# ccalantzis/BRDF

Hardware: AMD Instinct MI355X
Metric: BRDF residual-evals/sec (1 M samples, Ward 3-param), whole job; rel-err vs CPU levmar in `parity` (higher is better)
Workload: dtype f64

## Files before the change

brdf_amd/csrc/resident_fit_impl.h:

```cpp
#pragma once
#include <type_traits>

#if defined(BRDF_STAMPS)
#include <hip/hip_runtime.h>
static __device__ long long g_rlm_stamps[8];
static __device__ long long g_rlm_last;
#endif
#if defined(BRDF_STAMPS) && defined(__HIP_DEVICE_COMPILE__)
#define LM_STAMP(i) do { if (blockIdx.x == 0) { const long long now_ = clock64(); if ((i) != 0) g_rlm_stamps[i] += now_ - g_rlm_last; g_rlm_last = now_; } } while (0)
#endif
#include "batch_fit.h"
#include "stream_fit.h"

namespace brdf {

constexpr int kRThreads = 512;
constexpr int kRSpt = 8;
constexpr int kRTile = kRThreads * kRSpt;
constexpr int kRCap = kRTile;
constexpr int kRowWords = 2 * kSlots;
constexpr int kRowStride = 256;
constexpr int kRedCols = kRThreads / 4;
constexpr long long kSpinBudgetTicks = 200000000LL;

typedef unsigned long long u64;

struct ResidentCtl {
  unsigned abort;
  unsigned domain_bad;
  unsigned pad[30];
};

struct ResidentCtx {
  const double *c0, *c1, *c2, *x;
  u64 *rows;
  u64 *groups;
  ResidentCtl *ctl;
  unsigned launch_id;
  double p0[kM], opts[5], lb[kM], ub[kM], dscl[kM];
  int itmax, has_opts, has_lb, has_ub, has_dscl, want_covar, multi, analytic;
  int chain;
  int spec_jac;
  int dif_fused;
  Mailbox *mbox;
  int n;
  unsigned tag_base;
  long long spin_ticks;
  int sabotage_epoch;
  int replicas;
  long long *trace;
  int trace_epoch;
};

template <int METHOD>
using RMachine = typename std::conditional<METHOD == 0, DifMachine<kM>, typename std::conditional<METHOD == 1, BcMachine<kM>, DerMachine<kM>>::type>::type;

__device__ __forceinline__ double read_lane(double v, int lane) {
  const int lo = __builtin_amdgcn_readlane(__double2loint(v), lane);
  const int hi = __builtin_amdgcn_readlane(__double2hiint(v), lane);
  return __hiloint2double(hi, lo);
}

__device__ __forceinline__ void acc_normal_eq_fma(const double *j, double e, double *jtj6, double *jte3) {
  jtj6[0] = fma(j[0], j[0], jtj6[0]);
  jtj6[1] = fma(j[0], j[1], jtj6[1]);
  jtj6[2] = fma(j[1], j[1], jtj6[2]);
  jtj6[3] = fma(j[0], j[2], jtj6[3]);
  jtj6[4] = fma(j[1], j[2], jtj6[4]);
  jtj6[5] = fma(j[2], j[2], jtj6[5]);
  jte3[0] = fma(j[0], e, jte3[0]);
  jte3[1] = fma(j[1], e, jte3[1]);
  jte3[2] = fma(j[2], e, jte3[2]);
}
__device__ __forceinline__ double div_by(double x, double d, double r) {
  const double q = x * r;
  return fma(fma(-q, d, x), r, q);
}

#ifdef BRDF_STAMPS
#define RSTAMP(i) do { const long long now_ = clock64(); st_[i] += now_ - last_; last_ = now_; } while (0)
#define RTRACE(ctx_, epoch_, slot_, val_) do { if ((ctx_).trace && (int)(epoch_) == (ctx_).trace_epoch && (threadIdx.x & 63) == 0) (ctx_).trace[blockIdx.x * 8 + (slot_)] = (long long)(val_); } while (0)
#else
#define RSTAMP(i) do {} while (0)
#define RTRACE(ctx_, epoch_, slot_, val_) do {} while (0)
#endif

constexpr int kFc0 = 0, kFx = 1, kFq1 = 2, kFq2 = 3, kFhx = 4, kFwrk = 5, kFtb = 6;
template <int METHOD>
constexpr int sample_fields() { return METHOD == 0 ? 7 : 4; }

template <int METHOD>
struct RegSamples {
  static constexpr bool kUnrolled = true;
  double v[sample_fields<METHOD>()][kRSpt];
  __device__ __forceinline__ double get(int f, int k) const { return v[f][k]; }
  __device__ __forceinline__ void set(int f, int k, double x) { v[f][k] = x; }
};
template <int METHOD>
struct LdsSamples {
  static constexpr bool kUnrolled = false;
  double *base;
  __device__ __forceinline__ double get(int f, int k) const { return base[(f * kRSpt + k) * kWave]; }
  __device__ __forceinline__ void set(int f, int k, double x) { base[(f * kRSpt + k) * kWave] = x; }
};

template <bool UNROLLED, class F>
__device__ __forceinline__ void for_samples(int nk, F &&f) {
  if constexpr (UNROLLED) {
#pragma unroll
    for (int k = 0; k < kRSpt; ++k)
      if (k < nk) f(k);
  } else {
#pragma unroll 2
    for (int k = 0; k < nk; ++k) f(k);
  }
}

constexpr int kGroup = 16;
constexpr int kMaxGroups = 16;
constexpr int kReplicas = 8;
constexpr size_t kBlockGranules = (size_t)kRowWords * kGroup;
constexpr size_t kRowsGranules = 2 * (size_t)kMaxGroups * kBlockGranules;
constexpr size_t kGroupsGranules = 2 * (size_t)kReplicas * kBlockGranules;

typedef unsigned int u32x4 __attribute__((ext_vector_type(4)));
constexpr int kCacheSc1 = 16;
__device__ __forceinline__ __amdgpu_buffer_rsrc_t table_rsrc(const u64 *p, size_t granules) {
  return __builtin_amdgcn_make_buffer_rsrc(const_cast<u64 *>(p), 0, (int)(granules * sizeof(u64)), 0x00027000);
}
__device__ __forceinline__ void put_cell(__amdgpu_buffer_rsrc_t t, unsigned cell, unsigned tag, double v) {
  const u32x4 d = {(unsigned)__double2loint(v), tag, (unsigned)__double2hiint(v), tag};
  __builtin_amdgcn_raw_buffer_store_b128(d, t, (int)(cell * 16u), 0, kCacheSc1);
}

struct RowPublish {
  const u64 *rows;
  unsigned cell0;
  unsigned tag;
  bool on;
  bool withhold;
};

template <int NS, bool MAX = true, bool PUB = false>
__device__ __forceinline__ void worker_reduce(const double *acc, double mx, double *buf, double *out, const RowPublish &pub, long long *st_,
                                              long long &last_) {
  const int lane = threadIdx.x & (kWave - 1);
  const int wave = threadIdx.x >> 6;
  double v[NS + 1];
#pragma unroll
  for (int k = 0; k < NS; ++k) {
    double t = acc[k];
    t = t + dpp_move<0x111, 0xf, 0xf>(t, 0.0);
    t = t + dpp_move<0x112, 0xf, 0xf>(t, 0.0);
    v[k] = t;
  }
  if constexpr (MAX) {
    double t = mx;
    t = fmax(t, dpp_move<0x111, 0xf, 0xf>(t, 0.0));
    t = fmax(t, dpp_move<0x112, 0xf, 0xf>(t, 0.0));
    v[NS] = t;
  }
  constexpr int NV = NS + (MAX ? 1 : 0);
  if ((threadIdx.x & 3) == 3) {
#pragma unroll
    for (int k = 0; k < NV; ++k) buf[k * kRedCols + (threadIdx.x >> 2)] = v[k];
  }
  __syncthreads();
  RSTAMP(6);
  {
    constexpr int NW = kRThreads / kWave;
    const int k0 = wave, k1 = wave + NW;
    const bool has0 = k0 < NV, has1 = k1 < NV;
    double s0 = 0.0, s1 = 0.0;
    if (has0) {
      const double *src = buf + k0 * kRedCols;
      s0 = (k0 < NS || !MAX) ? src[lane] + src[lane + kWave] : fmax(src[lane], src[lane + kWave]);
    }
    if (has1) {
      const double *src = buf + k1 * kRedCols;
      s1 = (k1 < NS || !MAX) ? src[lane] + src[lane + kWave] : fmax(src[lane], src[lane + kWave]);
    }
    const bool max0 = MAX && has0 && k0 == NS, max1 = MAX && has1 && k1 == NS;
    if (!max0 && !max1) {
      wave_reduce2_to_last<OpSum, OpSum>(s0, s1);
    } else if (max1) {
      wave_reduce2_to_last<OpSum, OpMax>(s0, s1);
    } else {
      wave_reduce2_to_last<OpMax, OpSum>(s0, s1);
    }
    if constexpr (PUB) {
      if (pub.on) {
        if (lane == kWave - 1 && !pub.withhold) {
          const __amdgpu_buffer_rsrc_t rows = table_rsrc(pub.rows, kRowsGranules);
          if (has0) put_cell(rows, pub.cell0 + (max0 ? kSums : k0) * kGroup, pub.tag, s0);
          if (has1) put_cell(rows, pub.cell0 + (max1 ? kSums : k1) * kGroup, pub.tag, s1);
        }
        return;
      }
    }
    if (lane == kWave - 1) {
      if (has0) out[max0 ? kSums : k0] = s0;
      if (has1) out[max1 ? kSums : k1] = s1;
    }
  }
  __syncthreads();
}

__device__ __forceinline__ RowPublish row_publish(const ResidentCtx &ctx, unsigned epoch) {
  const unsigned grp = blockIdx.x / kGroup;
  return RowPublish{ctx.rows, ((epoch & 1u) * kMaxGroups + grp) * (kSlots * kGroup) + blockIdx.x % kGroup, ctx.tag_base + epoch + 1u, gridDim.x > 1,
                    (int)epoch == ctx.sabotage_epoch && blockIdx.x == gridDim.x - 1};
}

template <int NS, bool MAX = true>
__device__ __forceinline__ constexpr bool slot_used(int v) { return v < NS || (MAX && v == kSums); }

template <int NS, bool MAX = true, class Ctx>
__device__ __forceinline__ bool gather_block(const Ctx &ctx, __amdgpu_buffer_rsrc_t t, unsigned first, unsigned tag, int ncols,
                                             double (&val)[4], unsigned *polls) {
  const int lane = threadIdx.x & (kWave - 1);
  const int col = lane & 15, r = lane >> 4;
  const long long t0 = (long long)wall_clock64();
  for (unsigned spins = 0;; ++spins) {
    u32x4 d[4];
    bool ready = true;
#pragma unroll
    for (int j = 0; j < 4; ++j) {
      d[j] = u32x4{0u, tag, 0u, tag};
      if ((4 * j < NS) || (MAX && 4 * j <= kSums && kSums < 4 * j + 4)) {
        const int v = 4 * j + r;
        if (slot_used<NS, MAX>(v) && col < ncols) d[j] = __builtin_amdgcn_raw_buffer_load_b128(t, (int)((first + v * kGroup + col) * 16u), 0, kCacheSc1);
      }
    }
#pragma unroll
    for (int j = 0; j < 4; ++j) ready = ready && d[j].y == tag && d[j].w == tag;
    if (__all(ready)) {
#pragma unroll
      for (int j = 0; j < 4; ++j) val[j] = __hiloint2double((int)d[j].z, (int)d[j].x);
      *polls = spins;
      return true;
    }
    if ((spins & 63u) == 63u) {
      if (__hip_atomic_load(&ctx.ctl->abort, __ATOMIC_RELAXED, __HIP_MEMORY_SCOPE_AGENT) == ctx.launch_id ||
          (long long)wall_clock64() - t0 > ctx.spin_ticks) {
        __hip_atomic_store(&ctx.ctl->abort, ctx.launch_id, __ATOMIC_RELAXED, __HIP_MEMORY_SCOPE_AGENT);
        return false;
      }
    }
    __builtin_amdgcn_s_sleep(1);
  }
}

template <int NS, bool MAX>
__device__ __forceinline__ void fold_block(double (&val)[4]) {
  const int r = (int)(threadIdx.x & (kWave - 1)) >> 4;
  double mx = 0.0;
  if constexpr (MAX) mx = row_reduce_to_last<OpMax>(val[kSums / 4]);
#pragma unroll
  for (int j = 0; j < 4; ++j)
    if ((4 * j < NS) || (MAX && j == kSums / 4)) val[j] = row_reduce_to_last<OpSum>(val[j]);
  if (MAX && r == (kSums & 3)) val[kSums / 4] = mx;
}

template <int NS, bool MAX = true, bool PUBLISHED = false, class Ctx>
__device__ __forceinline__ bool control_exchange(const Ctx &ctx, unsigned epoch, double *sums, int *s_abort,
                                                 long long *st_, long long &last_) {
  const int lane = threadIdx.x & (kWave - 1);
  const int col = lane & 15, r = lane >> 4;
  const int G = gridDim.x;
  const int grp = blockIdx.x / kGroup, ngrp = (G + kGroup - 1) / kGroup;
  const int members = min(kGroup, G - grp * kGroup);
  const int leader = grp * kGroup + (grp & 7) % members;
  const unsigned tag = ctx.tag_base + epoch + 1u;
  constexpr unsigned kBlockCells = kSlots * kGroup;
  const __amdgpu_buffer_rsrc_t rows = table_rsrc(ctx.rows, kRowsGranules), groups = table_rsrc(ctx.groups, kGroupsGranules);
  const unsigned my_rows = ((epoch & 1u) * kMaxGroups + grp) * kBlockCells;
  const unsigned my_groups = (epoch & 1u) * kReplicas * kBlockCells;
  if constexpr (!PUBLISHED) {
    const bool withhold = (int)epoch == ctx.sabotage_epoch && blockIdx.x == gridDim.x - 1;
    if (slot_used<NS, MAX>(lane) && lane <= kSums && !withhold) put_cell(rows, my_rows + lane * kGroup + blockIdx.x % kGroup, tag, sums[lane]);
  }

  double val[4];
  unsigned polls = 0;
  if ((int)blockIdx.x == leader) {
    if (!gather_block<NS, MAX>(ctx, rows, my_rows, tag, members, val, &polls)) {
      *s_abort = 1;
      return false;
    }
#ifndef BRDF_TRACE_WORKERS
    RTRACE(ctx, epoch, 6, polls + 1);
#endif
    fold_block<NS, MAX>(val);
#pragma unroll
    for (int j = 0; j < 4; ++j) {
      const double t = dpp_move<0x15F, 0xf, 0xf>(val[j], 0.0);
      const int v = 4 * j + r;
      if (slot_used<NS, MAX>(v) && col < ctx.replicas) put_cell(groups, my_groups + col * kBlockCells + v * kGroup + grp, tag, t);
    }
  }
  RSTAMP(2);
  RTRACE(ctx, epoch, 3, wall_clock64());
  if (!gather_block<NS, MAX>(ctx, groups, my_groups + (blockIdx.x % ctx.replicas) * kBlockCells, tag, ngrp, val, &polls)) {
    *s_abort = 1;
    return false;
  }
  fold_block<NS, MAX>(val);
#pragma unroll
  for (int j = 0; j < 4; ++j) {
    const int v = 4 * j + r;
    if (slot_used<NS, MAX>(v) && col == kGroup - 1) sums[v] = val[j];
  }
  __builtin_amdgcn_fence(__ATOMIC_RELEASE, "wavefront");
  __builtin_amdgcn_wave_barrier();
  RSTAMP(3);
  RTRACE(ctx, epoch, 4, wall_clock64());
#ifndef BRDF_TRACE_WORKERS
  RTRACE(ctx, epoch, 7, polls);
#endif
  return true;
}

template <int MODEL>
__device__ __forceinline__ void build_uniforms_wave(PassUniforms<MODEL> &u, const Request<kM> &r, bool need_base, bool analytic_jac) {
  using Mdl = BrdfModel<MODEL>;
  const int lane = (int)(threadIdx.x & (kWave - 1));
  if (r.kind == RQ_EVAL_MULTI) {
    u.ncand = r.nk;
    u.analytic = analytic_jac ? 1 : 0;
    if (lane < kMaxCand && lane < r.nk) {
      const double pk[kM] = {r.pk[lane][0], r.pk[lane][1], r.pk[lane][2]};
      u.lk[lane] = Mdl::lin(pk);
      u.nk[lane] = Mdl::nl(pk);
    }
    return;
  }
  if ((r.kind == RQ_JAC && !analytic_jac) || r.kind == RQ_DIF_JAC) {
    u.ncand = 0;
    u.analytic = 0;
    u.central = r.central;
    u.scal = r.scal;
    u.dp_l2 = r.dp_l2;
#pragma unroll
    for (int j = 0; j < kM; ++j) u.dp[j] = r.dp[j];
    if (lane < 1 + 2 * kM) {
      const int j = lane == 0 ? 0 : (lane - 1) % kM;
      const bool plus = lane >= 1 && lane <= kM, minus = lane > kM;
      double pp[kM];
#pragma unroll
      for (int i = 0; i < kM; ++i) {
        pp[i] = r.p[i];
        if (i == j && plus) pp[i] = r.p[i] + r.d[i];
        if (i == j && minus) pp[i] = r.p[i] - r.d[i];
      }
      const Lin l = Mdl::lin(pp);
      const Nl nn = Mdl::nl(pp);
      if (lane == 0) {
        u.l0 = l;
        u.n0 = nn;
      } else if (plus) {
        u.lp[j] = l;
        if (j == kM - 1) u.np2 = nn;
        double dj = r.d[0];
#pragma unroll
        for (int i = 1; i < kM; ++i)
          if (i == j) dj = r.d[i];
        u.dinv[j] = (r.central ? 0.5 : 1.0) / dj;
      } else {
        u.lm[j] = l;
        if (j == kM - 1) u.nm2 = nn;
      }
    }
    return;
  }
  u.build(r, need_base, analytic_jac);
}

template <int MODEL, int METHOD, bool FAST, class Store>
__device__ __forceinline__ void sweep_pass(int kind, const PassUniforms<MODEL> &u, Store &st, double *jl, int tid, int nk, int nfull, unsigned okm,
                                           bool pend, const double *dpp, double *acc, double &mx) {
  constexpr bool U = Store::kUnrolled;
  constexpr bool W2 = BrdfModel<MODEL>::prep_planes == 2;
  auto prep = [&](int k) { return Prep{st.get(kFq1, k), W2 ? st.get(kFq2, k) : 0.0}; };
  auto dead = [&](int k) { return k >= nfull && !(okm >> k & 1u); };
  switch (kind) {
  case RQ_EVAL:
    if constexpr (METHOD != 0) {
      const EvalUniforms eu{scalar_copy(u.l0), scalar_copy(u.n0), 1.0};
      for_samples<U>(nk, [&](int k) {
        const double f = model_value<MODEL, FAST>(eu, st.get(kFc0, k), prep(k));
        double e = st.get(kFx, k) - f;
        if (dead(k)) e = 0.0;
        acc[0] = fma(e, e, acc[0]);
        mx = fmax(mx, fabs(e));
      });
    }
    break;
  case RQ_SCALED:
    if constexpr (METHOD != 0) {
      const EvalUniforms eu{scalar_copy(u.l0), scalar_copy(u.n0), scalar_copy(u.scal)};
      for_samples<U>(nk, [&](int k) {
        const double f = model_value<MODEL, FAST>(eu, st.get(kFc0, k), prep(k));
        double t = (st.get(kFx, k) - f) / eu.scal;
        if (dead(k)) t = 0.0;
        acc[0] = fma(t, t, acc[0]);
      });
    }
    break;
  case RQ_EVAL_MULTI:
    if constexpr (METHOD != 2) {
      if (u.ncand == kMaxCand) {
        if constexpr (METHOD == 0) {
          for_samples<U>(nk, [&](int k) {
            const double c0 = st.get(kFc0, k), x = st.get(kFx, k);
            const Prep q = prep(k);
            const bool d = dead(k);
#pragma unroll
            for (int j0 = 0; j0 < kMaxCand; j0 += 4) {
              double e[4];
#pragma unroll
              for (int j = 0; j < 4; ++j) e[j] = x - model_value_k<MODEL, FAST>(u, j0 + j, c0, q);
#pragma unroll
              for (int j = 0; j < 4; ++j) {
                if (d) e[j] = 0.0;
                acc[j0 + j] = fma(e[j], e[j], acc[j0 + j]);
              }
            }
          });
          break;
        }
#pragma unroll
        for (int j0 = 0; j0 < kMaxCand; j0 += 4) {
          Lin l4[4];
          Nl n4[4];
#pragma unroll
          for (int j = 0; j < 4; ++j) {
            l4[j] = scalar_copy(u.lk[j0 + j]);
            n4[j] = scalar_copy(u.nk[j0 + j]);
          }
          for_samples<U>(nk, [&](int k) {
            const double c0 = st.get(kFc0, k), x = st.get(kFx, k);
            const Prep q = prep(k);
            const bool d = dead(k);
            double e[4];
#pragma unroll
            for (int j = 0; j < 4; ++j) e[j] = x - BrdfModel<MODEL>::combine(l4[j], c0, BrdfModel<MODEL>::template shape<FAST>(n4[j], c0, q));
#pragma unroll
            for (int j = 0; j < 4; ++j) {
              if (d) e[j] = 0.0;
              acc[j0 + j] = fma(e[j], e[j], acc[j0 + j]);
            }
          });
        }
        break;
      }
      for_samples<U>(nk, [&](int k) {
        const double c0 = st.get(kFc0, k), x = st.get(kFx, k);
        const Prep q = prep(k);
#pragma unroll
        for (int j = 0; j < kMaxCand; ++j)
          if (j < u.ncand) {
            double e = x - model_value_k<MODEL, FAST>(u, j, c0, q);
            if (dead(k)) e = 0.0;
            acc[j] = fma(e, e, acc[j]);
          }
      });
    }
    break;
  case RQ_JAC:
    if constexpr (METHOD != 0) {
      auto jac = [&](auto jk) {
        constexpr int JK = decltype(jk)::value;
        JacUniforms ju;
        ju.l0 = scalar_copy(u.l0);
        ju.n0 = scalar_copy(u.n0);
        ju.analytic = JK == 2;
        ju.central = JK == 1;
        if (JK == 2) {
          ju.an[0] = scalar_copy(u.an[0]);
          ju.an[1] = scalar_copy(u.an[1]);
        } else {
#pragma unroll
          for (int j = 0; j < kM; ++j) {
            ju.lp[j] = scalar_copy(u.lp[j]);
            ju.dinv[j] = scalar_copy(u.dinv[j]);
            if (JK == 1) ju.lm[j] = scalar_copy(u.lm[j]);
          }
          ju.np2 = scalar_copy(u.np2);
          if (JK == 1) ju.nm2 = scalar_copy(u.nm2);
        }
        for_samples<U>(nk, [&](int k) {
          double f0 = 0.0, j[kM];
          if (JK == 2)
            model_an_row<MODEL, FAST>(ju, st.get(kFc0, k), prep(k), f0, j);
          else if (JK == 1)
            model_fd_row_t<MODEL, FAST, true>(ju, st.get(kFc0, k), prep(k), true, f0, 0.0, false, j);
          else
            model_fd_row_t<MODEL, FAST, false>(ju, st.get(kFc0, k), prep(k), true, f0, 0.0, false, j);
          double e = st.get(kFx, k) - f0;
          if (dead(k)) e = j[0] = j[1] = j[2] = 0.0;
          acc_normal_eq_fma(j, e, acc, acc + kNL);
          acc[kNL + kM] = fma(e, e, acc[kNL + kM]);
        });
      };
      if (u.analytic)
        jac(std::integral_constant<int, 2>{});
      else if (u.central)
        jac(std::integral_constant<int, 1>{});
      else
        jac(std::integral_constant<int, 0>{});
    }
    break;
  case RQ_DIF_INIT:
    if constexpr (METHOD == 0) {
      for_samples<U>(nk, [&](int k) {
        const double h = model_value<MODEL, FAST>(u, st.get(kFc0, k), prep(k));
        st.set(kFhx, k, h);
        double e = st.get(kFx, k) - h;
        if (dead(k)) e = 0.0;
        acc[0] = fma(e, e, acc[0]);
      });
    }
    break;
  case RQ_DIF_JAC:
    if constexpr (METHOD == 0) {
      for_samples<U>(nk, [&](int k) {
        const int s = k * kRThreads + tid;
        const double h = st.get(kFhx, k);
        double f0 = 0.0, j[kM];
        model_fd_row<MODEL, FAST>(u, st.get(kFc0, k), prep(k), false, f0, h, true, j);
        double e = st.get(kFx, k) - h;
        if (dead(k)) e = j[0] = j[1] = j[2] = 0.0;
        jl[s] = j[0];
        jl[kRCap + s] = j[1];
        jl[2 * kRCap + s] = j[2];
        acc_normal_eq_fma(j, e, acc, acc + kNL);
      });
    }
    break;
  case RQ_DIF_TRIAL:
    if constexpr (METHOD == 0) {
      struct TrialUniforms {
        Lin lq;
        Nl nq;
        double dp[kM], dp_l2;
      };
      TrialUniforms tu;
      tu.lq = scalar_copy(u.lq);
      tu.nq = scalar_copy(u.nq);
#pragma unroll
      for (int j = 0; j < kM; ++j) tu.dp[j] = scalar_copy(u.dp[j]);
      tu.dp_l2 = scalar_copy(u.dp_l2);
      const double dpp_s[kM] = {scalar_copy(dpp[0]), scalar_copy(dpp[1]), scalar_copy(dpp[2])};
      const TrialUniforms &u = tu;
      const double *dpp = dpp_s;
      const double rinv = 1.0 / u.dp_l2;
      auto value_q = [&](int k) { return model_value_q<MODEL, FAST>(u, st.get(kFc0, k), prep(k)); };
      auto body = [&](int k, const double w) {
        const int s = k * kRThreads + tid;
        const double h = st.get(kFhx, k), x = st.get(kFx, k);
        double jo[kM] = {jl[s], jl[kRCap + s], jl[2 * kRCap + s]};
        if (pend) {
          const double tp = st.get(kFtb, k);
#pragma unroll
          for (int j = 0; j < kM; ++j) jo[j] = fma(tp, dpp[j], jo[j]);
          jl[s] = jo[0];
          jl[kRCap + s] = jo[1];
          jl[2 * kRCap + s] = jo[2];
        }
        double t = jo[0] * u.dp[0], jn[kM];
        t = fma(jo[1], u.dp[1], t);
        t = fma(jo[2], u.dp[2], t);
        t = div_by(w - h - t, u.dp_l2, rinv);
#pragma unroll
        for (int j = 0; j < kM; ++j) jn[j] = fma(t, u.dp[j], jo[j]);
        double en = x - w, eo = x - h;
        if (dead(k)) en = eo = jn[0] = jn[1] = jn[2] = t = 0.0;
        st.set(kFwrk, k, w);
        st.set(kFtb, k, t);
        acc[0] = fma(en, en, acc[0]);
#pragma unroll
        for (int j = 0; j < kM; ++j) acc[1 + j] = fma(jo[j], t, acc[1 + j]);
        acc[1 + kM] = fma(t, t, acc[1 + kM]);
#pragma unroll
        for (int j = 0; j < kM; ++j) acc[2 + kM + j] = fma(jn[j], en, acc[2 + kM + j]);
        acc[2 + 2 * kM] = fma(t, eo, acc[2 + 2 * kM]);
      };
      for_samples<U>(nk, [&](int k) { body(k, value_q(k)); });
    }
    break;
  default: break;
  }
}

template <int METHOD, bool PUB = false>
__device__ __forceinline__ void reduce_pass(int kind, const double *acc, double mx, double *red, double *sums, const RowPublish &pub, long long *st_,
                                            long long &last_) {
  if constexpr (METHOD == 0) {
    switch (kind) {
    case RQ_DIF_JAC: worker_reduce<SumLayout<kM>::DIF_JAC, false, PUB>(acc, mx, red, sums, pub, st_, last_); break;
    case RQ_DIF_TRIAL: worker_reduce<kTrialSums, false, PUB>(acc, mx, red, sums, pub, st_, last_); break;
    case RQ_EVAL_MULTI: worker_reduce<kMaxCand, false, PUB>(acc, mx, red, sums, pub, st_, last_); break;
    default: worker_reduce<1, false, PUB>(acc, mx, red, sums, pub, st_, last_); break;
    }
  } else {
    switch (kind) {
    case RQ_JAC: worker_reduce<SumLayout<kM>::JAC, false, PUB>(acc, mx, red, sums, pub, st_, last_); break;
    case RQ_EVAL_MULTI: worker_reduce<kMaxCand, false, PUB>(acc, mx, red, sums, pub, st_, last_); break;
    default: worker_reduce<1, METHOD == 1, PUB>(acc, mx, red, sums, pub, st_, last_); break;
    }
  }
}

#define RESIDENT_KERNEL_HEAD                                      \
  template <int MODEL, int METHOD, bool FAST, bool BATCHED>       \
  __global__ __launch_bounds__(kRThreads) void resident_fit_kernel(ResidentCtx ctx, BatchCtx bctx)
#define RESIDENT_KERNEL_FLAGS constexpr bool RAGGED = false;
#define RESIDENT_KERNEL_COUNT(fit_, stride_) (stride_)
#include "resident_fit_kernel.inc"
#undef RESIDENT_KERNEL_HEAD
#undef RESIDENT_KERNEL_FLAGS
#undef RESIDENT_KERNEL_COUNT

#define RESIDENT_KERNEL_HEAD                          \
  template <int MODEL, int METHOD, bool FAST>         \
  __global__ __launch_bounds__(kRThreads) void resident_fit_ragged_kernel(ResidentCtx ctx, RaggedBatchCtx bctx)
#define RESIDENT_KERNEL_FLAGS constexpr bool BATCHED = true, RAGGED = true;
#define RESIDENT_KERNEL_COUNT(fit_, stride_) ragged_count(bctx.counts, (fit_), (stride_))
#include "resident_fit_kernel.inc"
#undef RESIDENT_KERNEL_HEAD
#undef RESIDENT_KERNEL_FLAGS
#undef RESIDENT_KERNEL_COUNT

using ResidentKernelFn = void (*)(ResidentCtx, BatchCtx);
using ResidentRaggedFn = void (*)(ResidentCtx, RaggedBatchCtx);
constexpr int kFastPath = 0, kExactPath = 1;
struct ResidentKernels {
  ResidentKernelFn single[2], batched[2];
  ResidentRaggedFn ragged[2];
#ifdef BRDF_STAMPS
  void (*take_lm_stamps)(long long *out8);
#endif
};

template <int MODEL, int METHOD, bool FAST, bool BATCHED>
constexpr ResidentKernelFn resident_kernel() {
  if constexpr (FAST || MODEL != MODEL_WARD)
    return resident_fit_kernel<MODEL, METHOD, FAST, BATCHED>;
  else
    return nullptr;
}

template <int MODEL, int METHOD, bool FAST>
constexpr ResidentRaggedFn resident_ragged_kernel() {
  if constexpr (FAST || MODEL != MODEL_WARD)
    return resident_fit_ragged_kernel<MODEL, METHOD, FAST>;
  else
    return nullptr;
}

#ifdef BRDF_STAMPS
static void take_lm_stamps(long long *out8) {
  const long long zero[8] = {0, 0, 0, 0, 0, 0, 0, 0};
  (void)hipMemcpyFromSymbol(out8, HIP_SYMBOL(g_rlm_stamps), sizeof zero);
  (void)hipMemcpyToSymbol(HIP_SYMBOL(g_rlm_stamps), zero, sizeof zero);
}
#define BRDF_RESIDENT_STAMPS_ENTRY , take_lm_stamps
#else
#define BRDF_RESIDENT_STAMPS_ENTRY
#endif

#define BRDF_RESIDENT_INSTANCE(MODEL_, METHOD_, NAME_)                                                                      \
  ResidentKernels resident_kernels_##NAME_() {                                                                              \
    return {{resident_kernel<MODEL_, METHOD_, true, false>(), resident_kernel<MODEL_, METHOD_, false, false>()},            \
            {resident_kernel<MODEL_, METHOD_, true, true>(), resident_kernel<MODEL_, METHOD_, false, true>()},              \
            {resident_ragged_kernel<MODEL_, METHOD_, true>(), resident_ragged_kernel<MODEL_, METHOD_, false>()} BRDF_RESIDENT_STAMPS_ENTRY}; \
  }

}
```

brdf_amd/csrc/resident_fit_kernel.inc:

```
RESIDENT_KERNEL_HEAD {
  RESIDENT_KERNEL_FLAGS
  using Machine = RMachine<METHOD>;
  using Mdl = BrdfModel<MODEL>;
  constexpr int NF = sample_fields<METHOD>();
  constexpr bool kControlFromLds = (METHOD == 0) || (METHOD == 1 && !BATCHED);
  static_assert(sizeof(Machine) % 4 == 0, "machine copied as dwords");
  __shared__ Machine sm;
  __shared__ PassUniforms<MODEL> su;
  __shared__ double red[kSlots * kRedCols];
  __shared__ double sums[kSlots];
  __shared__ double dp_prev[kM + 1];
  __shared__ int s_abort, s_bad;
  __shared__ double cst[kControlFromLds ? NF * kRSpt * kWave : 2];
  constexpr int kJl = (METHOD == 0) ? 3 * kRCap : 2;
  __shared__ double jl[kJl];

  const int tid = threadIdx.x;
  const int wave = __builtin_amdgcn_readfirstlane((int)threadIdx.x >> 6);
  const int G = BATCHED ? 1 : (int)gridDim.x;
  const int fit = blockIdx.x;
  const int stride = BATCHED ? bctx.n : ctx.n;
  const int n = RESIDENT_KERNEL_COUNT(fit, stride);
  if constexpr (BATCHED && !FAST) {
    if (bctx.flags[fit] != kNeedsExact) return;
  }

  if (wave == 0) {
    double p0[kM], opts[5], lb[kM], ub[kM], dscl[kM];
    int itmax, has_opts, has_lb, has_ub, has_dscl = 0, want_covar = 0, multi, analytic, chain, spec_jac;
    if constexpr (BATCHED) {
#pragma unroll
      for (int i = 0; i < kM; ++i) {
        p0[i] = bctx.p[(size_t)fit * kM + i];
        lb[i] = bctx.lb[i];
        ub[i] = bctx.ub[i];
        dscl[i] = 1.0;
      }
#pragma unroll
      for (int i = 0; i < 5; ++i) opts[i] = bctx.opts[i];
      itmax = bctx.itmax, has_opts = bctx.has_opts, has_lb = bctx.has_lb, has_ub = bctx.has_ub, multi = bctx.multi, analytic = bctx.analytic;
      chain = bctx.chain, spec_jac = bctx.spec_jac;
    } else {
#pragma unroll
      for (int i = 0; i < kM; ++i) {
        p0[i] = ctx.p0[i];
        lb[i] = ctx.lb[i];
        ub[i] = ctx.ub[i];
        dscl[i] = ctx.dscl[i];
      }
#pragma unroll
      for (int i = 0; i < 5; ++i) opts[i] = ctx.opts[i];
      itmax = ctx.itmax, has_opts = ctx.has_opts, has_lb = ctx.has_lb, has_ub = ctx.has_ub, has_dscl = ctx.has_dscl;
      want_covar = ctx.want_covar, multi = ctx.multi, analytic = ctx.analytic, chain = ctx.chain, spec_jac = ctx.spec_jac;
    }
    const double *po = has_opts ? opts : nullptr;
    if constexpr (METHOD == 0) {
      sm.start(p0, n, itmax, po, want_covar, 1, chain);
    } else if constexpr (METHOD == 1) {
      sm.start(p0, n, has_lb ? lb : nullptr, has_ub ? ub : nullptr, has_dscl ? dscl : nullptr, itmax, po, want_covar, multi, BATCHED ? 0 : spec_jac);
      sm.c.analytic_jac = analytic;
    } else {
      sm.start(p0, n, itmax, po, want_covar);
    }
    (void)analytic, (void)chain, (void)spec_jac;
  }
  if (tid == 0) s_abort = s_bad = 0;
  if (tid <= kM) dp_prev[tid] = 0.0;
  __syncthreads();
  if (wave == 0) {
    if constexpr (METHOD == 1)
      su.build(sm.h.req, true, sm.c.analytic_jac != 0);
    else
      su.build(sm.h.req, true, METHOD == 2);
  }

  int vb = BATCHED ? 0 : (int)blockIdx.x;
  if (!BATCHED && (G & 7) == 0) vb = (blockIdx.x & 7) * (G >> 3) + (blockIdx.x >> 3);
  const int tile = (n + G - 1) / G;
  const int begin = vb * tile;
  const int end = min(n, begin + tile);
  const double *pc0 = BATCHED ? bctx.angles + (size_t)fit * 3 * stride : ctx.c0;
  const double *pc1 = BATCHED ? pc0 + stride : ctx.c1;
  const double *pc2 = BATCHED ? pc0 + 2 * (size_t)stride : ctx.c2;
  const double *px = BATCHED ? bctx.x + (size_t)fit * stride : ctx.x;
  const int nk = (tile + kRThreads - 1) / kRThreads;
  const int nfull = max(end - begin, 0) / kRThreads;
  RegSamples<METHOD> rs;
  LdsSamples<METHOD> ls{cst + (tid & (kWave - 1))};
  unsigned okm = 0;
  {
    bool bad = false;
#pragma unroll
    for (int k = 0; k < kRSpt; ++k) {
      const int i = begin + tid + k * kRThreads;
      const bool ok = i < end;
      okm |= ok ? (1u << k) : 0u;
      const int ii = ok ? i : begin;
      const double r0 = pc0[ii];
      const double r1 = Mdl::uses_c1 ? pc1[ii] : 0.0;
      const double r2 = Mdl::uses_c2 ? pc2[ii] : 0.0;
      const Prep q = Mdl::template prepare<FAST>(r0, r1, r2);
      rs.v[kFc0][k] = r0;
      rs.v[kFx][k] = px[ii];
      rs.v[kFq1][k] = q.q1;
      rs.v[kFq2][k] = q.q2;
      if constexpr (METHOD == 0) rs.v[kFhx][k] = rs.v[kFwrk][k] = rs.v[kFtb][k] = 0.0;
      if (FAST && ok && !Mdl::domain_ok(r0, r1, r2)) bad = true;
    }
    if constexpr (BATCHED) {
      if (FAST && bad) s_bad = 1;
    } else {
      if (FAST && bad) __hip_atomic_store(&ctx.ctl->domain_bad, ctx.launch_id, __ATOMIC_RELAXED, __HIP_MEMORY_SCOPE_AGENT);
    }
    if (kControlFromLds && wave == 0) {
#pragma unroll
      for (int f = 0; f < NF; ++f)
#pragma unroll
        for (int k = 0; k < kRSpt; ++k) ls.set(f, k, rs.v[f][k]);
    }
  }
  __syncthreads();

  constexpr bool kPub = !BATCHED;
  auto row_pub = [&](unsigned epoch) {
    if constexpr (kPub)
      return row_publish(ctx, epoch);
    else
      return RowPublish{nullptr, 0u, 0u, false, false};
  };
  int cur_sel_hx = 0, cur_sel_j = 0;
  auto decisions = [&](auto &st, bool &pend) {
    pend = false;
    if constexpr (METHOD == 0) {
      pend = sm.h.req.sel_j != cur_sel_j;
      if (pend && sm.h.req.kind != RQ_DIF_TRIAL) pend = false;
      cur_sel_j = sm.h.req.sel_j;
      if (sm.h.req.sel_hx != cur_sel_hx) {
        for_samples<std::remove_reference<decltype(st)>::type::kUnrolled>(nk, [&](int k) { st.set(kFhx, k, st.get(kFwrk, k)); });
        cur_sel_hx = sm.h.req.sel_hx;
      }
    }
  };

  if (wave == 0) {
    long long st_[8] = {0, 0, 0, 0, 0, 0, 0, 0};
    long long last_ = clock64();
    long long n_jac = 0;
    typename Machine::Cold cold0;
    typename std::conditional<METHOD == 0, typename DifMachine<kM>::CoreInts, int>::type ints_regs{};
    if constexpr (METHOD == 0) {
      cold0.itmax = lm_uniform(sm.c.itmax);
      cold0.n = lm_uniform(sm.c.n);
      cold0.want_covar = lm_uniform(sm.c.want_covar);
      cold0.refresh = lm_uniform(sm.c.refresh);
      cold0.speculative = lm_uniform(sm.c.speculative);
      cold0.multi = lm_uniform(sm.c.multi);
      cold0.o.forward = lm_uniform(sm.c.o.forward);
      cold0.o.tau = scalar_copy(sm.c.o.tau);
      cold0.o.eps1 = scalar_copy(sm.c.o.eps1);
      cold0.o.eps2 = scalar_copy(sm.c.o.eps2);
      cold0.o.eps2sq = scalar_copy(sm.c.o.eps2sq);
      cold0.o.eps3 = scalar_copy(sm.c.o.eps3);
      cold0.o.delta = scalar_copy(sm.c.o.delta);
      ints_regs = sm.h;
      Machine::uniform_ints(ints_regs);
    }
    const int fused = (METHOD == 0) ? (BATCHED ? bctx.dif_fused : ctx.dif_fused) : 0;
    int n_fused = 0;
    (void)cold0, (void)ints_regs, (void)fused;
    const long long t_first = (long long)wall_clock64();
    unsigned epoch = 0;
    for (;; ++epoch) {
      const int kind = sm.h.req.kind;
      if (kind == RQ_DONE) break;
      if (kind == RQ_JAC || kind == RQ_DIF_JAC) ++n_jac;
      RTRACE(ctx, epoch, 0, wall_clock64());
      {
        bool pend;
        double acc[kSums];
#pragma unroll
        for (int k = 0; k < kSums; ++k) acc[k] = 0.0;
        double mx = 0.0;
        const double dpp[kM] = {dp_prev[0], dp_prev[1], dp_prev[2]};
        if constexpr (kControlFromLds) {
          decisions(ls, pend);
          sweep_pass<MODEL, METHOD, FAST>(kind, su, ls, jl, tid, nk, nfull, okm, pend, dpp, acc, mx);
        } else {
          decisions(rs, pend);
          sweep_pass<MODEL, METHOD, FAST>(kind, su, rs, jl, tid, nk, nfull, okm, pend, dpp, acc, mx);
        }
        RSTAMP(5);
        RTRACE(ctx, epoch, 1, wall_clock64());
        reduce_pass<METHOD, kPub>(kind, acc, mx, red, sums, row_pub(epoch), st_, last_);
      }
      RSTAMP(1);
      RTRACE(ctx, epoch, 2, wall_clock64());
      bool alive = true;
      if constexpr (BATCHED && FAST) {
        if (epoch == 0) {
          if (s_bad) {
            if (tid == 0) bctx.flags[fit] = kNeedsExact;
            s_abort = 1;
            alive = false;
          } else if (tid == 0) {
            bctx.flags[fit] = 0;
          }
        }
      }
      if constexpr (!BATCHED) {
       if (gridDim.x > 1) {
        if constexpr (METHOD == 0) {
          switch (kind) {
          case RQ_DIF_JAC: alive = control_exchange<SumLayout<kM>::DIF_JAC, false, kPub>(ctx, epoch, sums, &s_abort, st_, last_); break;
          case RQ_DIF_TRIAL: alive = control_exchange<kTrialSums, false, kPub>(ctx, epoch, sums, &s_abort, st_, last_); break;
          case RQ_EVAL_MULTI: alive = control_exchange<kMaxCand, false, kPub>(ctx, epoch, sums, &s_abort, st_, last_); break;
          default: alive = control_exchange<1, false, kPub>(ctx, epoch, sums, &s_abort, st_, last_); break;
          }
        } else {
          switch (kind) {
          case RQ_JAC: alive = control_exchange<SumLayout<kM>::JAC, false, kPub>(ctx, epoch, sums, &s_abort, st_, last_); break;
          case RQ_EVAL_MULTI: alive = control_exchange<kMaxCand, false, kPub>(ctx, epoch, sums, &s_abort, st_, last_); break;
          default: alive = control_exchange<1, METHOD == 1, kPub>(ctx, epoch, sums, &s_abort, st_, last_); break;
          }
        }
       }
      }
      if (!alive) {
        __syncthreads();
        return;
      }
      bool stepped = false;
      constexpr bool kTrialFromRegs = METHOD == 0 && !BATCHED;
      if (kind == RQ_DIF_TRIAL) {
        if constexpr (METHOD == 0) {
          if (fused) {
            if constexpr (kTrialFromRegs) {
              const bool took = fused_trial_step_split_device<Machine>(
                  cold0, ints_regs, static_cast<typename Machine::CoreReals &>(sm.h), sm.h.cool, sm.h.req, sums, su.dp, [&](const typename Machine::TrialCommit &late) {
#pragma unroll
                    for (int j = 0; j < kM; ++j) dp_prev[j] = su.dp[j];
                    dp_prev[kM] = su.dp_l2;
                    RSTAMP(7);
                    su.build_trial(late.pdp, late.dp, late.dp_l2, false);
                    RTRACE(ctx, epoch, 5, wall_clock64());
                    __syncthreads();
                    RSTAMP(4);
                  });
              if (took) {
                ++n_fused;
                Machine::uniform_ints(ints_regs);
                continue;
              }
            } else {
              stepped = fused_trial_step_device<Machine>(cold0, ints_regs, static_cast<typename Machine::CoreReals &>(sm.h), sm.h.cool, sm.h.req, sums, su.dp);
              if (stepped) {
                ++n_fused;
                Machine::uniform_ints(ints_regs);
              }
            }
          }
          if (!stepped) expand_trial_sums(static_cast<const typename Machine::Core &>(sm.h), sm.h.cool, su.dp, sums);
        }
#pragma unroll
        for (int j = 0; j < kM; ++j) dp_prev[j] = su.dp[j];
        dp_prev[kM] = su.dp_l2;
      }
      if (!stepped) {
        if constexpr (METHOD == 0) {
          typename Machine::Cold cc;
          cc.itmax = cold0.itmax, cc.n = cold0.n, cc.want_covar = cold0.want_covar, cc.refresh = cold0.refresh;
          cc.speculative = cold0.speculative, cc.multi = cold0.multi, cc.o = cold0.o;
          for (int i = 0; i < kInfoSz; ++i) cc.info[i] = 0.0;
          for (int i = 0; i < kM * kM; ++i) cc.covar[i] = 0.0;
          cc.ret = kLmError;
          Machine::template run<true, true>(cc, ints_regs, static_cast<typename Machine::CoreReals &>(sm.h), sm.h.cool, sm.h.req, sums, sums[kSums]);
          Machine::uniform_ints(ints_regs);
          if (sm.h.req.kind == RQ_DONE) {
            for (int i = 0; i < kInfoSz; ++i) sm.c.info[i] = cc.info[i];
            for (int i = 0; i < kM * kM; ++i) sm.c.covar[i] = cc.covar[i];
            sm.c.ret = cc.ret;
          }
        } else
        if constexpr (METHOD == 1)
          sm.template step<true, true, false, !BATCHED>(sums, sums[kSums]);
        else
          sm.template step<true>(sums, sums[kSums]);
      }
      RSTAMP(7);
      if (sm.h.req.kind != RQ_DONE) {
        if constexpr (METHOD == 1 && !BATCHED)
          build_uniforms_wave(su, sm.h.req, false, sm.c.analytic_jac != 0);
        else if constexpr (METHOD == 1)
          su.build(sm.h.req, false, sm.c.analytic_jac != 0);
        else
          su.build(sm.h.req, false, METHOD == 2);
      }
      RTRACE(ctx, epoch, 5, wall_clock64());
      __syncthreads();
      RSTAMP(4);
    }
    if constexpr (BATCHED) {
      if constexpr (RAGGED && FAST) {
        if (epoch == 0 && tid == 0) bctx.flags[fit] = 0;
      }
      if (tid == 0) {
        double *po = bctx.p + (size_t)fit * kM;
        for (int i = 0; i < kM; ++i) po[i] = sm.h.p[i];
        if (bctx.info)
          for (int i = 0; i < kInfoSz; ++i) bctx.info[(size_t)fit * kInfoSz + i] = sm.c.info[i];
        if (bctx.ret) bctx.ret[fit] = sm.c.ret;
      }
      return;
    }
    if (blockIdx.x == 0 && tid == 0) {
      Mailbox *mb = ctx.mbox;
      mb->ret = sm.c.ret;
      mb->passes = (int)epoch;
      if constexpr (METHOD == 1)
        mb->infeasible_mask = sm.c.infeasible_mask;
      else
        mb->infeasible_mask = 0;
      mb->domain_bad = __hip_atomic_load(&ctx.ctl->domain_bad, __ATOMIC_RELAXED, __HIP_MEMORY_SCOPE_AGENT) == ctx.launch_id ? 1 : 0;
      mb->n_jac = n_jac;
      mb->n_eval = (long long)epoch - n_jac;
      mb->t_first = t_first;
      mb->t_last = (long long)wall_clock64();
      st_[0] = n_fused;
      for (int k = 0; k < 8; ++k) mb->stamps[k] = st_[k];
      for (int i = 0; i < kM; ++i) mb->p[i] = sm.h.p[i];
      for (int i = 0; i < kInfoSz; ++i) mb->info[i] = sm.c.info[i];
      for (int i = 0; i < kM * kM; ++i) mb->covar[i] = sm.c.covar[i];
      __threadfence_system();
      __hip_atomic_store(&mb->done, 1, __ATOMIC_RELEASE, __HIP_MEMORY_SCOPE_SYSTEM);
    }
    return;
  }

  long long wst_[8] = {0, 0, 0, 0, 0, 0, 0, 0}, wlast_ = 0;
  for (unsigned epoch = 0;; ++epoch) {
    const int kind = sm.h.req.kind;
    if (kind == RQ_DONE) break;
    bool pend;
    decisions(rs, pend);
    double acc[kSums];
#pragma unroll
    for (int k = 0; k < kSums; ++k) acc[k] = 0.0;
    double mx = 0.0;
    const double dpp[kM] = {dp_prev[0], dp_prev[1], dp_prev[2]};
    sweep_pass<MODEL, METHOD, FAST>(kind, su, rs, jl, tid, nk, nfull, okm, pend, dpp, acc, mx);
#ifdef BRDF_TRACE_WORKERS
    if constexpr (!BATCHED) {
      if (wave == 4) RTRACE(ctx, epoch, 6, wall_clock64());
      if (wave == 7) RTRACE(ctx, epoch, 7, wall_clock64());
    }
#endif
    reduce_pass<METHOD, kPub>(kind, acc, mx, red, sums, row_pub(epoch), wst_, wlast_);
    __syncthreads();
    if (s_abort) return;
  }
}
```

Measured before the change: 144.1 billion.

## Offload control wave's trial model evaluations to worker waves via LDS sharing

In the resident LM kernel for method 0, worker waves now compute the model values for the control wave's LDS-resident samples during the trial pass and write them into an extra LDS plane. They signal completion through a workgroup atomic counter. The control wave spins on that counter with a timeout and then uses the precomputed values instead of evaluating the model itself. The aim is to shorten the control wave's critical-path sweep, which gates every epoch. In exchange it adds LDS use, spin-wait synchronisation, and an abort path if the wait times out.

```diff
diff --git a/brdf_amd/csrc/resident_fit_impl.h b/brdf_amd/csrc/resident_fit_impl.h
--- a/brdf_amd/csrc/resident_fit_impl.h
+++ b/brdf_amd/csrc/resident_fit_impl.h
@@ -86,6 +86,7 @@
 #endif
 
 constexpr int kFc0 = 0, kFx = 1, kFq1 = 2, kFq2 = 3, kFhx = 4, kFwrk = 5, kFtb = 6;
+constexpr int kFval = 7;
 template <int METHOD>
 constexpr int sample_fields() { return METHOD == 0 ? 7 : 4; }
 
@@ -376,9 +377,30 @@
   u.build(r, need_base, analytic_jac);
 }
 
-template <int MODEL, int METHOD, bool FAST, class Store>
+struct NoTrialShare {
+  static constexpr bool kOn = false;
+};
+struct TrialShare {
+  static constexpr bool kOn = true;
+  double *cst;
+  unsigned *count;
+  int wave;
+  unsigned expect;
+  long long spin_ticks;
+  bool failed;
+};
+constexpr int kShareWaves = kRThreads / kWave - 1;
+constexpr int kShareSlot7Wave = 4;
+#ifdef CSHARE_SLOTS
+constexpr int kShareSlots = CSHARE_SLOTS;
+#else
+constexpr int kShareSlots = kRSpt;
+#endif
+static_assert(kRSpt == kShareWaves + 1 && kShareSlot7Wave - 1 + (kRSpt - kShareSlot7Wave) == kRSpt - 1, "slots 0..7 are all taken");
+
+template <int MODEL, int METHOD, bool FAST, class Store, class Share = NoTrialShare>
 __device__ __forceinline__ void sweep_pass(int kind, const PassUniforms<MODEL> &u, Store &st, double *jl, int tid, int nk, int nfull, unsigned okm,
-                                           bool pend, const double *dpp, double *acc, double &mx) {
+                                           bool pend, const double *dpp, double *acc, double &mx, Share &&sh = Share{}) {
   constexpr bool U = Store::kUnrolled;
   constexpr bool W2 = BrdfModel<MODEL>::prep_planes == 2;
   auto prep = [&](int k) { return Prep{st.get(kFq1, k), W2 ? st.get(kFq2, k) : 0.0}; };
@@ -586,7 +608,77 @@
         for (int j = 0; j < kM; ++j) acc[2 + kM + j] = fma(jn[j], en, acc[2 + kM + j]);
         acc[2 + 2 * kM] = fma(t, eo, acc[2 + 2 * kM]);
       };
-      for_samples<U>(nk, [&](int k) { body(k, value_q(k)); });
+      if constexpr (std::remove_reference<Share>::type::kOn) {
+        const int lane = tid & (kWave - 1);
+        if constexpr (U) {
+#ifdef CSHARE_INTERLEAVE
+          {
+            const int hk0 = sh.wave - 1;
+            double *c0p = sh.cst + (hk0 < nk ? hk0 : 0) * kWave + lane;
+            const Prep q0{c0p[kFq1 * kRSpt * kWave], W2 ? c0p[kFq2 * kRSpt * kWave] : 0.0};
+            const double hv = model_value_q<MODEL, FAST>(u, c0p[kFc0 * kRSpt * kWave], q0);
+            const double w0 = value_q(0);
+            if (hk0 < nk) c0p[kFval * kRSpt * kWave] = hv;
+            if (sh.wave == kShareSlot7Wave && kRSpt - 1 < nk) {
+              double *c = sh.cst + (kRSpt - 1) * kWave + lane;
+              const Prep q{c[kFq1 * kRSpt * kWave], W2 ? c[kFq2 * kRSpt * kWave] : 0.0};
+              c[kFval * kRSpt * kWave] = model_value_q<MODEL, FAST>(u, c[kFc0 * kRSpt * kWave], q);
+            }
+            __builtin_amdgcn_fence(__ATOMIC_RELEASE, "workgroup");
+            __builtin_amdgcn_wave_barrier();
+            if (lane == 0) __hip_atomic_fetch_add(sh.count, 1u, __ATOMIC_RELAXED, __HIP_MEMORY_SCOPE_WORKGROUP);
+            body(0, w0);
+#pragma unroll
+            for (int k = 1; k < kRSpt; ++k)
+              if (k < nk) body(k, value_q(k));
+          }
+#else
+#ifdef CSHARE_SLOT7_CONTROL
+          const int hstep = kRSpt;
+#else
+          const int hstep = sh.wave == kShareSlot7Wave ? kRSpt - kShareSlot7Wave : kRSpt;
+#endif
+#pragma unroll 1
+          for (int hk = sh.wave - 1; hk < min(nk, kShareSlots); hk += hstep) {
+            double *c = sh.cst + hk * kWave + lane;
+            const Prep q{c[kFq1 * kRSpt * kWave], W2 ? c[kFq2 * kRSpt * kWave] : 0.0};
+            c[kFval * kRSpt * kWave] = model_value_q<MODEL, FAST>(u, c[kFc0 * kRSpt * kWave], q);
+          }
+#ifdef CSHARE_BARRIER
+          __syncthreads();
+#else
+          __builtin_amdgcn_fence(__ATOMIC_RELEASE, "workgroup");
+          __builtin_amdgcn_wave_barrier();
+          if (lane == 0) __hip_atomic_fetch_add(sh.count, 1u, __ATOMIC_RELAXED, __HIP_MEMORY_SCOPE_WORKGROUP);
+#endif
+          for_samples<U>(nk, [&](int k) { body(k, value_q(k)); });
+#endif
+        } else {
+#ifdef CSHARE_SLOT7_CONTROL
+          if (kShareWaves < nk) st.set(kFval, kShareWaves, value_q(kShareWaves));
+#endif
+#ifdef CSHARE_BARRIER
+          __syncthreads();
+#else
+          const long long t0 = (long long)wall_clock64();
+          for (unsigned spins = 0; __hip_atomic_load(sh.count, __ATOMIC_RELAXED, __HIP_MEMORY_SCOPE_WORKGROUP) != sh.expect; ++spins) {
+            if ((spins & 255u) == 255u && (long long)wall_clock64() - t0 > sh.spin_ticks) {
+              sh.failed = true;
+              break;
+            }
+            __builtin_amdgcn_s_sleep(1);
+          }
+          __builtin_amdgcn_fence(__ATOMIC_ACQUIRE, "workgroup");
+#endif
+#ifdef CSHARE_SLOTS
+          for_samples<U>(nk, [&](int k) { body(k, k < kShareSlots ? st.get(kFval, k) : value_q(k)); });
+#else
+          for_samples<U>(nk, [&](int k) { body(k, st.get(kFval, k)); });
+#endif
+        }
+      } else {
+        for_samples<U>(nk, [&](int k) { body(k, value_q(k)); });
+      }
     }
     break;
   default: break;
diff --git a/brdf_amd/csrc/resident_fit_kernel.inc b/brdf_amd/csrc/resident_fit_kernel.inc
--- a/brdf_amd/csrc/resident_fit_kernel.inc
+++ b/brdf_amd/csrc/resident_fit_kernel.inc
@@ -11,9 +11,11 @@
   __shared__ double sums[kSlots];
   __shared__ double dp_prev[kM + 1];
   __shared__ int s_abort, s_bad;
-  __shared__ double cst[kControlFromLds ? NF * kRSpt * kWave : 2];
+  constexpr bool kHelp = METHOD == 0 && !BATCHED;
+  __shared__ double cst[kControlFromLds ? (NF + (kHelp ? 1 : 0)) * kRSpt * kWave : 2];
   constexpr int kJl = (METHOD == 0) ? 3 * kRCap : 2;
   __shared__ double jl[kJl];
+  __shared__ unsigned s_help;
 
   const int tid = threadIdx.x;
   const int wave = __builtin_amdgcn_readfirstlane((int)threadIdx.x >> 6);
@@ -65,6 +67,9 @@
     (void)analytic, (void)chain, (void)spec_jac;
   }
   if (tid == 0) s_abort = s_bad = 0;
+  if constexpr (kHelp) {
+    if (tid == 0) s_help = 0u;
+  }
   if (tid <= kM) dp_prev[tid] = 0.0;
   __syncthreads();
   if (wave == 0) {
@@ -167,7 +172,9 @@
     }
     const int fused = (METHOD == 0) ? (BATCHED ? bctx.dif_fused : ctx.dif_fused) : 0;
     int n_fused = 0;
-    (void)cold0, (void)ints_regs, (void)fused;
+    int n_trial = 0;
+    int share_failed = 0;
+    (void)cold0, (void)ints_regs, (void)fused, (void)n_trial, (void)share_failed;
     const long long t_first = (long long)wall_clock64();
     unsigned epoch = 0;
     for (;; ++epoch) {
@@ -182,7 +189,18 @@
         for (int k = 0; k < kSums; ++k) acc[k] = 0.0;
         double mx = 0.0;
         const double dpp[kM] = {dp_prev[0], dp_prev[1], dp_prev[2]};
-        if constexpr (kControlFromLds) {
+        if constexpr (kHelp) {
+          decisions(ls, pend);
+          n_trial = lm_uniform(n_trial + (kind == RQ_DIF_TRIAL ? 1 : 0));
+          TrialShare sh{cst, &s_help, 0, (unsigned)(kShareWaves * n_trial), ctx.spin_ticks, false};
+          sweep_pass<MODEL, METHOD, FAST>(kind, su, ls, jl, tid, nk, nfull, okm, pend, dpp, acc, mx, sh);
+          share_failed = lm_uniform(sh.failed ? 1 : 0);
+          if (share_failed) {
+            s_abort = 1;
+            __hip_atomic_store(&ctx.ctl->abort, ctx.launch_id, __ATOMIC_RELAXED, __HIP_MEMORY_SCOPE_AGENT);
+            __threadfence();
+          }
+        } else if constexpr (kControlFromLds) {
           decisions(ls, pend);
           sweep_pass<MODEL, METHOD, FAST>(kind, su, ls, jl, tid, nk, nfull, okm, pend, dpp, acc, mx);
         } else {
@@ -195,7 +213,16 @@
       }
       RSTAMP(1);
       RTRACE(ctx, epoch, 2, wall_clock64());
+#ifdef BRDF_TRACE_WORKERS
+      RTRACE(ctx, epoch, 2, kind);
+#endif
       bool alive = true;
+      if constexpr (kHelp) {
+        if (share_failed) {
+          __syncthreads();
+          return;
+        }
+      }
       if constexpr (BATCHED && FAST) {
         if (epoch == 0) {
           if (s_bad) {
@@ -312,6 +339,9 @@
       }
       return;
     }
+    if constexpr (kHelp) {
+      if (blockIdx.x == 0 && __hip_atomic_load(&ctx.ctl->abort, __ATOMIC_RELAXED, __HIP_MEMORY_SCOPE_AGENT) == ctx.launch_id) return;
+    }
     if (blockIdx.x == 0 && tid == 0) {
       Mailbox *mb = ctx.mbox;
       mb->ret = sm.c.ret;
@@ -347,7 +377,12 @@
     for (int k = 0; k < kSums; ++k) acc[k] = 0.0;
     double mx = 0.0;
     const double dpp[kM] = {dp_prev[0], dp_prev[1], dp_prev[2]};
-    sweep_pass<MODEL, METHOD, FAST>(kind, su, rs, jl, tid, nk, nfull, okm, pend, dpp, acc, mx);
+    if constexpr (kHelp) {
+      TrialShare sh{cst, &s_help, wave, 0u, 0, false};
+      sweep_pass<MODEL, METHOD, FAST>(kind, su, rs, jl, tid, nk, nfull, okm, pend, dpp, acc, mx, sh);
+    } else {
+      sweep_pass<MODEL, METHOD, FAST>(kind, su, rs, jl, tid, nk, nfull, okm, pend, dpp, acc, mx);
+    }
 #ifdef BRDF_TRACE_WORKERS
     if constexpr (!BATCHED) {
       if (wave == 4) RTRACE(ctx, epoch, 6, wall_clock64());
```

Result: slower. 141.9 billion (-1.5%).
